# nfmoore/databricks-kubernetes-mlops-poc

Measured on AMD Instinct MI355X. Metric: requests/sec (whole node), credit-default /score, bs=1024, higher is better.
Workload: dtype fp32; 1 GPU; model=RandomForest 500xdepth16 + IForest100 + TabularDrift, global_batch=1024, request_rows=1024, with_drift=True, train_rows=20000, parallelism=dp1, device=cuda

## Files before the change

csrc/creditcore_kernels.hip:

```cpp

#include <torch/extension.h>

#include <c10/hip/HIPGuard.h>
#include <c10/hip/HIPStream.h>
#include <hip/hip_runtime.h>

#define BLOCK 256
#define N_CAT 9
#define N_NUM 14
#define MAX_DRIFT_ROWS 16384
static constexpr size_t KS_LDS_BYTES_MAX = 160 * 1024 - 1024;

#define HIP_CHECK(expr)                                              \
  do {                                                               \
    hipError_t _e = (expr);                                          \
    TORCH_CHECK(_e == hipSuccess, "HIP error: ", hipGetErrorString(_e)); \
  } while (0)


template <bool DIRECT>
__global__ __launch_bounds__(BLOCK) void forest_kernel(
    const short* __restrict__ codes,
    const float* __restrict__ nums,
    const float* __restrict__ medians,
    const int4* __restrict__ nodes,
    const int* __restrict__ tree_off,
    int n_trees,
    const int* __restrict__ feat_col,
    const int* __restrict__ feat_code,
    int n_rows,
    double* __restrict__ acc)
{
  __shared__ short s_codes[N_CAT * BLOCK];
  __shared__ float s_nums[N_NUM * BLOCK];

  const int tid = threadIdx.x;
  const int row = blockIdx.x * BLOCK + tid;
  if (row < n_rows) {
    if (!DIRECT) {
#pragma unroll
      for (int c = 0; c < N_CAT; ++c) s_codes[c * BLOCK + tid] = codes[row * N_CAT + c];
    }
#pragma unroll
    for (int c = 0; c < N_NUM; ++c) {
      const float v = nums[row * N_NUM + c];
      s_nums[c * BLOCK + tid] = isnan(v) ? medians[c] : v;
    }
  }
  if (row >= n_rows) return;

  double local = 0.0;
  for (int t = blockIdx.y; t < n_trees; t += gridDim.y) {
    const int base = tree_off[t];
    int4 nd = nodes[base];
    while (nd.x >= 0) {
      float v;
      if (DIRECT) {
        v = s_nums[nd.x * BLOCK + tid];
      } else {
        const int col = feat_col[nd.x];
        const int code = feat_code[nd.x];
        v = (code >= 0) ? ((s_codes[col * BLOCK + tid] == (short)code) ? 1.0f : 0.0f)
                        : s_nums[col * BLOCK + tid];
      }
      const float thr = __int_as_float(nd.y);
      nd = nodes[base + ((v <= thr) ? nd.z : nd.w)];
    }
    local += (double)__int_as_float(nd.y);
  }
  atomicAdd(&acc[row], local);
}

template <bool DIRECT>
__global__ __launch_bounds__(BLOCK) void forest_kernel_ilp(
    const short* __restrict__ codes,
    const float* __restrict__ nums,
    const float* __restrict__ medians,
    const int4* __restrict__ nodes,
    const int* __restrict__ tree_off,
    int n_trees,
    const int* __restrict__ feat_col,
    const int* __restrict__ feat_code,
    int n_rows,
    double* __restrict__ acc)
{
  __shared__ short s_codes[N_CAT * BLOCK];
  __shared__ float s_nums[N_NUM * BLOCK];
  const int tid = threadIdx.x;
// ... 832 lines not shown
  for (int i = threadIdx.x; i < m; i += blockDim.x) {
    float v = nums[i * n_cols + j];
    if (isnan(v)) v = medians[j];
    s_vals[i] = v;
  }
  const int64_t ref_lo = rs_off[j];
  const int n = (int)(rs_off[j + 1] - ref_lo);
  const float* __restrict__ ref = ref_sorted + ref_lo;
  __syncthreads();

  const int per = (m + gridDim.y - 1) / gridDim.y;
  const int e0 = blockIdx.y * per;
  const int e1 = min(m, e0 + per);

  double dmax = 0.0;
  for (int i = e0 + threadIdx.x; i < e1; i += blockDim.x) {
    const float x = s_vals[i];
    int lt = 0, le = 0;
    int k = 0;
    for (; k + 3 < m; k += 4) {
      const float v0 = s_vals[k], v1 = s_vals[k + 1];
      const float v2 = s_vals[k + 2], v3 = s_vals[k + 3];
      lt += (int)(v0 < x) + (int)(v1 < x) + (int)(v2 < x) + (int)(v3 < x);
      le += (int)(v0 <= x) + (int)(v1 <= x) + (int)(v2 <= x) + (int)(v3 <= x);
    }
    for (; k < m; ++k) {
      const float v = s_vals[k];
      lt += (int)(v < x);
      le += (int)(v <= x);
    }
    int l = 0, r = n;
    while (l < r) {
      const int mid = (l + r) >> 1;
      if (ref[mid] < x) l = mid + 1; else r = mid;
    }
    const int sl = l;
    r = n;
    while (l < r) {
      const int mid = (l + r) >> 1;
      if (ref[mid] <= x) l = mid + 1; else r = mid;
    }
    const int sr = l;
    const double fl = fabs((double)sl / n - (double)lt / m);
    const double fr = fabs((double)sr / n - (double)le / m);
    dmax = fmax(dmax, fmax(fl, fr));
  }

#pragma unroll
  for (int off = 32; off > 0; off >>= 1)
    dmax = fmax(dmax, __shfl_down(dmax, off, 64));
  __syncthreads();
  float* s_red = s_vals;
  const int wave = threadIdx.x >> 6;
  if ((threadIdx.x & 63) == 0) s_red[wave] = (float)dmax;
  __syncthreads();
  if (threadIdx.x == 0) {
    float d = s_red[0];
    for (int w = 1; w < (int)(blockDim.x >> 6); ++w) d = fmaxf(d, s_red[w]);
    scratch[(int64_t)j * gridDim.y + blockIdx.y] = d;
  }
}

__global__ __launch_bounds__(64) void ks_count_reduce_kernel(
    const float* __restrict__ scratch,
    int g, int n_cols,
    float* __restrict__ ks_d)
{
  const int j = blockIdx.x * 64 + threadIdx.x;
  if (j >= n_cols) return;
  float d = 0.0f;
  for (int k = 0; k < g; ++k) d = fmaxf(d, scratch[(int64_t)j * g + k]);
  ks_d[j] = d;
}

inline int ks_mb_blocks(int b) {
  int g = (b + 127) / 128;
  if (g < 1) g = 1;
  if (g > 128) g = 128;
  return g;
}
constexpr int KS_MB_MAX_G = 128;


namespace {

inline int ceil_div(int a, int b) { return (a + b - 1) / b; }

void check_inputs(const torch::Tensor& codes, const torch::Tensor& nums) {
  TORCH_CHECK(codes.is_cuda() && nums.is_cuda(), "inputs must be on GPU");
  TORCH_CHECK(codes.scalar_type() == torch::kInt16, "codes must be int16");
  TORCH_CHECK(nums.scalar_type() == torch::kFloat32, "nums must be float32");
  TORCH_CHECK(codes.is_contiguous() && nums.is_contiguous(), "inputs must be contiguous");
  TORCH_CHECK(codes.size(1) == N_CAT && nums.size(1) == N_NUM, "bad feature counts");
  TORCH_CHECK(codes.size(0) == nums.size(0), "row count mismatch");
}

}

std::vector<torch::Tensor> score_forest_pipeline(
    torch::Tensor codes, torch::Tensor nums,
    torch::Tensor cls_nodes, torch::Tensor cls_off,
    torch::Tensor feat_col, torch::Tensor feat_code,
    torch::Tensor medians, int64_t n_onehot,
    torch::Tensor if_nodes, torch::Tensor if_off,
    double if_denom, double if_offset, double if_threshold)
{
  (void)n_onehot;
  check_inputs(codes, nums);
  const int B = (int)codes.size(0);
  const int t_cls = (int)cls_off.size(0) - 1;
  const int t_if = (int)if_off.size(0) - 1;

  auto opts_f64 = torch::TensorOptions().dtype(torch::kFloat64).device(codes.device());
  auto cls_acc = torch::zeros({B}, opts_f64);
  auto if_acc = torch::zeros({B}, opts_f64);
  auto proba = torch::empty({B}, opts_f64);
  auto iscore = torch::empty({B}, opts_f64);
  auto outlier = torch::empty({B}, opts_f64);

  hipStream_t stream = c10::hip::getCurrentHIPStream();
  const int row_blocks = ceil_div(B, BLOCK);
  auto tree_chunks = [&](int t) {
    int c = ceil_div(2048, row_blocks);
    return std::max(1, std::min(c, t));
  };

  dim3 g_cls(row_blocks, tree_chunks(t_cls));
  hipLaunchKernelGGL((forest_kernel<false>), g_cls, dim3(BLOCK), 0, stream,
      codes.data_ptr<short>(), nums.data_ptr<float>(), medians.data_ptr<float>(),
      reinterpret_cast<const int4*>(cls_nodes.data_ptr<int>()),
      cls_off.data_ptr<int>(), t_cls,
      feat_col.data_ptr<int>(), feat_code.data_ptr<int>(),
      B, cls_acc.data_ptr<double>());

  dim3 g_if(row_blocks, tree_chunks(t_if));
  hipLaunchKernelGGL((forest_kernel<true>), g_if, dim3(BLOCK), 0, stream,
      codes.data_ptr<short>(), nums.data_ptr<float>(), medians.data_ptr<float>(),
      reinterpret_cast<const int4*>(if_nodes.data_ptr<int>()),
      if_off.data_ptr<int>(), t_if,
      nullptr, nullptr,
      B, if_acc.data_ptr<double>());

  hipLaunchKernelGGL(finalize_kernel, dim3(row_blocks), dim3(BLOCK), 0, stream,
      cls_acc.data_ptr<double>(), if_acc.data_ptr<double>(), B,
      0, 1.0 / (double)t_cls, 0.0, if_denom, if_offset, if_threshold,
      proba.data_ptr<double>(), iscore.data_ptr<double>(), outlier.data_ptr<double>());
  HIP_CHECK(hipGetLastError());

  return {proba, iscore, outlier};
}

torch::Tensor forest_contrib(
    torch::Tensor codes, torch::Tensor nums,
    torch::Tensor cls_nodes, torch::Tensor cls_node_value,
    torch::Tensor cls_off,
    torch::Tensor feat_col, torch::Tensor feat_code,
    torch::Tensor medians, int64_t cls_kind, int64_t block_target)
{
  check_inputs(codes, nums);
  TORCH_CHECK(block_target >= 1 && block_target <= 65535, "bad block_target");
  auto on_dev = [&](const torch::Tensor& t, torch::ScalarType st, const char* name) {
    TORCH_CHECK(t.is_cuda() && t.device() == codes.device(), name,
                " must be on the inputs' GPU");
    TORCH_CHECK(t.scalar_type() == st && t.is_contiguous(), name,
                " has the wrong dtype or is not contiguous");
  };
// ... 1201 lines not shown
#pragma unroll
  for (int off = 32; off > 0; off >>= 1)
    dmax = fmax(dmax, __shfl_down(dmax, off, 64));
  if ((threadIdx.x & 63) == 0 && dmax > 0.0)
    atomicMax(&ks_bits[j], __float_as_uint((float)dmax));
}

torch::Tensor ks_stats_sorted(
    torch::Tensor xs_sorted, torch::Tensor ref_sorted, torch::Tensor rs_off)
{
  TORCH_CHECK(xs_sorted.is_cuda() && xs_sorted.scalar_type() == torch::kFloat32
              && xs_sorted.is_contiguous());
  const int F = (int)xs_sorted.size(0);
  const int B = (int)xs_sorted.size(1);
  TORCH_CHECK((int)rs_off.size(0) == F + 1, "rs_off size mismatch");
  auto bits = torch::zeros({F},
      torch::TensorOptions().dtype(torch::kInt32).device(xs_sorted.device()));
  hipStream_t stream = c10::hip::getCurrentHIPStream();
  auto rs_off64 = rs_off.to(torch::kInt64);
  hipLaunchKernelGGL(ks_scan_kernel, dim3(F, ceil_div(B, BLOCK)), dim3(BLOCK), 0, stream,
      xs_sorted.data_ptr<float>(), F, B,
      ref_sorted.data_ptr<float>(), rs_off64.data_ptr<int64_t>(),
      reinterpret_cast<unsigned int*>(bits.data_ptr<int>()));
  HIP_CHECK(hipGetLastError());
  return bits.view(torch::kFloat32);
}

torch::Tensor ks_stats(
    torch::Tensor nums, torch::Tensor medians,
    torch::Tensor ref_sorted, torch::Tensor rs_off,
    int64_t block, int64_t ref_lds)
{
  TORCH_CHECK(nums.is_cuda() && nums.scalar_type() == torch::kFloat32 && nums.is_contiguous());
  const int B = (int)nums.size(0);
  const int F = (int)nums.size(1);
  TORCH_CHECK(B <= MAX_DRIFT_ROWS, "K-S batch too large: ", B);
  TORCH_CHECK((int)rs_off.size(0) == F + 1, "rs_off size mismatch");
  TORCH_CHECK(block == 256 || block == 512, "block must be 256 or 512");
  auto ks_d = torch::empty({F},
      torch::TensorOptions().dtype(torch::kFloat32).device(nums.device()));
  hipStream_t stream = c10::hip::getCurrentHIPStream();
  int m_pow2 = (int)block / 64;
  while (m_pow2 < B) m_pow2 <<= 1;
  size_t smem = (size_t)m_pow2 * sizeof(float);
  auto rs_off64 = rs_off.to(torch::kInt64);
  if (ref_lds) {
    int64_t maxr = 0;
    auto ro = rs_off64.cpu();
    auto* rp = ro.data_ptr<int64_t>();
    for (int j = 0; j < F; ++j) maxr = std::max<int64_t>(maxr, rp[j + 1] - rp[j]);
    smem += (size_t)maxr * sizeof(float);
    TORCH_CHECK(smem <= KS_LDS_BYTES_MAX, "ref too large for LDS");
  }
  if (block == 512)
    hipLaunchKernelGGL((ks_kernel_t<512>), dim3(F), dim3(512), smem, stream,
        nums.data_ptr<float>(), medians.data_ptr<float>(), F, B, m_pow2,
        (int)ref_lds, ref_sorted.data_ptr<float>(),
        rs_off64.data_ptr<int64_t>(), ks_d.data_ptr<float>());
  else
    hipLaunchKernelGGL((ks_kernel_t<256>), dim3(F), dim3(256), smem, stream,
        nums.data_ptr<float>(), medians.data_ptr<float>(), F, B, m_pow2,
        (int)ref_lds, ref_sorted.data_ptr<float>(),
        rs_off64.data_ptr<int64_t>(), ks_d.data_ptr<float>());
  HIP_CHECK(hipGetLastError());
  return ks_d;
}


inline bool spin_sync_enabled() {
  static const bool on = (std::getenv("CREDITCORE_BLOCK_SYNC") == nullptr);
  return on;
}

inline void sync_stream(hipStream_t s) {
  if (spin_sync_enabled()) {
    hipError_t e;
    while ((e = hipStreamQuery(s)) == hipErrorNotReady) {}
    if (e != hipSuccess) HIP_CHECK(e);
  } else {
    HIP_CHECK(hipStreamSynchronize(s));
  }
}

inline void sync_event(hipEvent_t ev) {
  static const bool spin = (std::getenv("CREDITCORE_SPIN_EVENT") != nullptr);
  if (spin) {
    hipError_t e;
    while ((e = hipEventQuery(ev)) == hipErrorNotReady) {}
    if (e != hipSuccess) HIP_CHECK(e);
  } else {
    HIP_CHECK(hipEventSynchronize(ev));
  }
}

struct ScoreSession {
  torch::Tensor cls_nodes, cls_off, feat_col, feat_code, medians;
  torch::Tensor if_nodes, if_off, ref_sorted, rs_off, cat_off;
  torch::Tensor d_codes, d_nums, acc, outs, d_drift, d_ks_scratch;
  size_t drift_bytes = 0, drift_ksd_off = 0;
  torch::Tensor pin_codes, pin_nums, pin_outs, pin_drift;
  torch::Tensor pin_hist, pin_ksd;
  double if_denom{}, if_offset{}, if_threshold{};
  int cls_kind{};
  double cls_bias{};
  int64_t total_bins{}, t_cls{}, t_if{}, capacity{};
  int device_index{};
  hipStream_t stream{};
  hipStream_t stream2{};
  hipEvent_t ev_fork{}, ev_join{};
  hipEvent_t ev_done[2]{};

  int16_t* p_codes(int s) { return pin_codes.data_ptr<int16_t>() + (size_t)s * capacity * N_CAT; }
  float* p_nums(int s) { return pin_nums.data_ptr<float>() + (size_t)s * capacity * N_NUM; }
  double* p_outs(int s) { return pin_outs.data_ptr<double>() + (size_t)s * 3 * capacity; }
  uint8_t* p_drift(int s) { return pin_drift.data_ptr<uint8_t>() + (size_t)s * drift_bytes; }
  int32_t* p_hist(int s) { return reinterpret_cast<int32_t*>(p_drift(s)); }
  float* p_ksd(int s) { return reinterpret_cast<float*>(p_drift(s) + drift_ksd_off); }
  int32_t* d_hist() { return reinterpret_cast<int32_t*>(d_drift.data_ptr<uint8_t>()); }
  float* d_ksd() { return reinterpret_cast<float*>(d_drift.data_ptr<uint8_t>() + drift_ksd_off); }

  ScoreSession(py::dict model, int64_t cap, int dev) : capacity(cap), device_index(dev) {
    c10::hip::HIPGuard guard((c10::DeviceIndex)dev);
    auto devopt = torch::TensorOptions().device(torch::kCUDA, dev);
    auto up_i32 = [&](const char* k) {
      return py::cast<torch::Tensor>(model[k]).to(devopt.dtype(torch::kInt32)).contiguous();
    };
    auto up_f32 = [&](const char* k) {
      return py::cast<torch::Tensor>(model[k]).to(devopt.dtype(torch::kFloat32)).contiguous();
    };
    cls_nodes = up_i32("cls_nodes");
    cls_off = up_i32("cls_tree_offsets");
    feat_col = up_i32("feat_col");
    feat_code = up_i32("feat_code");
    medians = up_f32("medians");
    if_nodes = up_i32("if_nodes");
    if_off = up_i32("if_tree_offsets");
    ref_sorted = up_f32("ref_sorted");
    rs_off = py::cast<torch::Tensor>(model["ref_sorted_offsets"])
                 .to(devopt.dtype(torch::kInt64)).contiguous();
    cat_off = up_i32("ref_cat_offsets");
    if (model.contains("cls_kind")) cls_kind = py::cast<int>(model["cls_kind"]);
    if (model.contains("cls_bias")) cls_bias = py::cast<double>(model["cls_bias"]);
    if_denom = py::cast<double>(model["if_denom"]);
    if_offset = py::cast<double>(model["if_offset"]);
    if_threshold = py::cast<double>(model["if_threshold"]);
    t_cls = cls_off.size(0) - 1;
    t_if = if_off.size(0) - 1;
    total_bins = py::cast<torch::Tensor>(model["ref_cat_offsets"])[-1].item<int64_t>();

    d_codes = torch::empty({capacity, N_CAT}, devopt.dtype(torch::kInt16));
    d_nums = torch::empty({capacity, N_NUM}, devopt.dtype(torch::kFloat32));
    acc = torch::zeros({2, capacity}, devopt.dtype(torch::kFloat64));
    outs = torch::empty({3, capacity}, devopt.dtype(torch::kFloat64));
    drift_ksd_off = (size_t)total_bins * sizeof(int32_t);
    drift_bytes = drift_ksd_off + (size_t)N_NUM * sizeof(float);
    d_drift = torch::empty({(int64_t)drift_bytes}, devopt.dtype(torch::kUInt8));
    d_ks_scratch = torch::empty({(int64_t)N_NUM * KS_MB_MAX_G},
                                devopt.dtype(torch::kFloat32));

    auto pinned = torch::TensorOptions().pinned_memory(true);
    pin_codes = torch::empty({2, capacity, N_CAT}, pinned.dtype(torch::kInt16));
    pin_nums = torch::empty({2, capacity, N_NUM}, pinned.dtype(torch::kFloat32));
    pin_outs = torch::empty({2, 3, capacity}, pinned.dtype(torch::kFloat64));
    pin_drift = torch::empty({2, (int64_t)drift_bytes}, pinned.dtype(torch::kUInt8));
    pin_hist = pin_drift.slice(1, 0, (int64_t)drift_ksd_off).view(torch::kInt32);
    pin_ksd = pin_drift.slice(1, (int64_t)drift_ksd_off, (int64_t)drift_bytes)
                  .view(torch::kFloat32);

    auto rs = py::cast<torch::Tensor>(model["ref_sorted_offsets"]);
    auto rs_acc = rs.accessor<int32_t, 1>();
    for (int j = 0; j + 1 < rs.size(0); ++j)
      max_ref_len = std::max(max_ref_len, (int64_t)(rs_acc[j + 1] - rs_acc[j]));

    (void)hipFuncSetAttribute(reinterpret_cast<const void*>(&ks_kernel_t<256>),
        hipFuncAttributeMaxDynamicSharedMemorySize, (int)KS_LDS_BYTES);
    (void)hipFuncSetAttribute(reinterpret_cast<const void*>(&ks_kernel_t<512>),
        hipFuncAttributeMaxDynamicSharedMemorySize, (int)KS_LDS_BYTES);
    (void)hipFuncSetAttribute(
        reinterpret_cast<const void*>(&ks_count_mb_kernel_t<512>),
        hipFuncAttributeMaxDynamicSharedMemorySize, (int)KS_LDS_BYTES);

    HIP_CHECK(hipStreamCreateWithFlags(&stream, hipStreamNonBlocking));
    HIP_CHECK(hipStreamCreateWithFlags(&stream2, hipStreamNonBlocking));
    HIP_CHECK(hipEventCreateWithFlags(&ev_fork, hipEventDisableTiming));
    HIP_CHECK(hipEventCreateWithFlags(&ev_join, hipEventDisableTiming));
    HIP_CHECK(hipEventCreateWithFlags(&ev_done[0], hipEventDisableTiming));
    HIP_CHECK(hipEventCreateWithFlags(&ev_done[1], hipEventDisableTiming));
    HIP_CHECK(hipDeviceSynchronize());
  }

  ~ScoreSession() {
    if (stream) {
      (void)hipStreamSynchronize(stream);
      for (auto& kv : graphs) (void)hipGraphExecDestroy(kv.second);
      (void)hipStreamDestroy(stream);
      (void)hipStreamDestroy(stream2);
      (void)hipEventDestroy(ev_fork);
      (void)hipEventDestroy(ev_join);
      (void)hipEventDestroy(ev_done[0]);
      (void)hipEventDestroy(ev_done[1]);
    }
  }

  void record(int b, bool with_drift, int slot) {
    HIP_CHECK(hipMemcpyAsync(d_codes.data_ptr(), p_codes(slot),
        (size_t)b * N_CAT * sizeof(short), hipMemcpyHostToDevice, stream));
    HIP_CHECK(hipMemcpyAsync(d_nums.data_ptr(), p_nums(slot),
        (size_t)b * N_NUM * sizeof(float), hipMemcpyHostToDevice, stream));
    const bool fork_drift = with_drift && b > 64;
    hipStream_t sdrift = fork_drift ? stream2 : stream;
    if (fork_drift) {
      HIP_CHECK(hipEventRecord(ev_fork, stream));
      HIP_CHECK(hipStreamWaitEvent(stream2, ev_fork, 0));
    }
    double* acc_cls = acc.data_ptr<double>();
    double* acc_if = acc_cls + b;

    const int row_blocks = ceil_div(b, BLOCK);
    auto chunks = [&](int64_t t) {
      return std::max(1, std::min(ceil_div(2048, row_blocks), (int)((t + 1) / 2)));
    };
    const int c_cls = chunks(t_cls);
    const int c_if = chunks(t_if);
    hipLaunchKernelGGL(forest_kernel_dual, dim3(row_blocks, c_cls + c_if),
        dim3(BLOCK), 0, stream,
        d_codes.data_ptr<short>(), d_nums.data_ptr<float>(), medians.data_ptr<float>(),
        reinterpret_cast<const int4*>(cls_nodes.data_ptr<int>()),
        cls_off.data_ptr<int>(), (int)t_cls,
        feat_col.data_ptr<int>(), feat_code.data_ptr<int>(),
        reinterpret_cast<const int4*>(if_nodes.data_ptr<int>()),
        if_off.data_ptr<int>(), (int)t_if, c_cls, b, acc_cls, acc_if);

    double* proba = outs.data_ptr<double>();
    hipLaunchKernelGGL(finalize_kernel, dim3(row_blocks), dim3(BLOCK), 0, stream,
        acc_cls, acc_if, b, cls_kind, 1.0 / (double)t_cls, cls_bias,
        if_denom, if_offset, if_threshold,
        proba, proba + b, proba + 2 * b);

    if (with_drift) {
      const int hist_blocks = (b <= 2048) ? 1 : std::min(row_blocks, 1024);
      if (hist_blocks > 1)
        HIP_CHECK(hipMemsetAsync(d_hist(), 0, (size_t)total_bins * sizeof(int), sdrift));
      hipLaunchKernelGGL(cat_hist_kernel, dim3(hist_blocks), dim3(BLOCK),
          (size_t)total_bins * sizeof(int), sdrift,
          d_codes.data_ptr<short>(), b, cat_off.data_ptr<int>(), (int)total_bins,
          d_hist());
      if (b <= KS_COUNT_MAX_ROWS) {
        const size_t smem = (size_t)std::max(b, 512 / 64) * sizeof(float);
        hipLaunchKernelGGL((ks_count_kernel_t<512>), dim3(N_NUM), dim3(512),
            smem, sdrift,
            d_nums.data_ptr<float>(), medians.data_ptr<float>(), N_NUM, b,
            ref_sorted.data_ptr<float>(), rs_off.data_ptr<int64_t>(), d_ksd());
      } else if (std::getenv("CREDITCORE_KS_BITONIC") != nullptr) {
        int m_pow2 = 512 / 64;
        while (m_pow2 < b) m_pow2 <<= 1;
        hipLaunchKernelGGL((ks_kernel_t<512>), dim3(N_NUM), dim3(512),
            (size_t)m_pow2 * sizeof(float), sdrift,
            d_nums.data_ptr<float>(), medians.data_ptr<float>(), N_NUM, b,
            m_pow2, 0, ref_sorted.data_ptr<float>(),
            rs_off.data_ptr<int64_t>(), d_ksd());
      } else {
        const int g = ks_mb_blocks(b);
        const size_t smem = (size_t)std::max(b, 512 / 64) * sizeof(float);
        hipLaunchKernelGGL((ks_count_mb_kernel_t<512>), dim3(N_NUM, g),
            dim3(512), smem, sdrift,
            d_nums.data_ptr<float>(), medians.data_ptr<float>(), N_NUM, b,
            ref_sorted.data_ptr<float>(), rs_off.data_ptr<int64_t>(),
            d_ks_scratch.data_ptr<float>());
        hipLaunchKernelGGL(ks_count_reduce_kernel, dim3(1), dim3(64), 0,
            sdrift, d_ks_scratch.data_ptr<float>(), g, N_NUM, d_ksd());
      }
      HIP_CHECK(hipMemcpyAsync(p_drift(slot), d_drift.data_ptr<uint8_t>(),
          drift_bytes, hipMemcpyDeviceToHost, sdrift));
      if (fork_drift) HIP_CHECK(hipEventRecord(ev_join, sdrift));
    }
    HIP_CHECK(hipMemcpyAsync(p_outs(slot), proba,
        (size_t)(3 * b) * sizeof(double), hipMemcpyDeviceToHost, stream));
    if (fork_drift) HIP_CHECK(hipStreamWaitEvent(stream, ev_join, 0));
    HIP_CHECK(hipGetLastError());
  }

  void score(int64_t b64, bool with_drift, bool sync, int64_t slot64) {
    TORCH_CHECK(b64 >= 1 && b64 <= capacity, "batch out of range: ", b64);
    TORCH_CHECK(!with_drift || b64 <= MAX_DRIFT_ROWS, "drift batch too large: ", b64);
    TORCH_CHECK(slot64 == 0 || slot64 == 1, "slot must be 0/1");
    const int b = (int)b64;
    const int slot = (int)slot64;
    py::gil_scoped_release nogil;
    c10::hip::HIPGuard guard((c10::DeviceIndex)device_index);

    const uint64_t key = ((uint64_t)b << 2) | ((with_drift ? 1u : 0u) << 1) | (uint64_t)slot;
    const bool graphable = ((b & (b - 1)) == 0) || (b % 256 == 0);
    auto it = graphs.find(key);
    if (it == graphs.end()) {
      if (!graphable || graphs.size() >= 128) {
        record(b, with_drift, slot);
        if (sync) sync_stream(stream);
        else HIP_CHECK(hipEventRecord(ev_done[slot], stream));
        return;
      }
      hipGraph_t graph;
      HIP_CHECK(hipStreamBeginCapture(stream, hipStreamCaptureModeThreadLocal));
      record(b, with_drift, slot);
      HIP_CHECK(hipStreamEndCapture(stream, &graph));
      hipGraphExec_t exec;
      HIP_CHECK(hipGraphInstantiate(&exec, graph, nullptr, nullptr, 0));
      HIP_CHECK(hipGraphDestroy(graph));
      it = graphs.emplace(key, exec).first;
    }
    HIP_CHECK(hipGraphLaunch(it->second, stream));
    if (sync) sync_stream(stream);
    else HIP_CHECK(hipEventRecord(ev_done[slot], stream));
  }

  void wait_slot(int64_t slot) {
    py::gil_scoped_release nogil;
    sync_event(ev_done[slot & 1]);
  }

  std::unordered_map<uint64_t, hipGraphExec_t> graphs;
  int64_t max_ref_len{};
  static constexpr size_t KS_LDS_BYTES = KS_LDS_BYTES_MAX;

  void synchronize() {
    py::gil_scoped_release nogil;
    HIP_CHECK(hipStreamSynchronize(stream));
  }
};


#include <pybind11/numpy.h>

#include <cmath>
#include <string>
#include <unordered_map>
#include <vector>

namespace py = pybind11;

py::tuple encode_records(py::list recs, py::list vocabs, py::list cat_names,
                         py::list num_names, py::str missing_cat) {
  const ssize_t b = py::len(recs);
  const int ncat = (int)py::len(cat_names);
  const int nnum = (int)py::len(num_names);
  py::array_t<int16_t> codes({b, (ssize_t)ncat});
  py::array_t<float> nums({b, (ssize_t)nnum});
  auto* cp = codes.mutable_data();
  auto* fp = nums.mutable_data();

  std::vector<std::unordered_map<std::string, int16_t>> maps(ncat);
  std::vector<int16_t> missing_code(ncat, -1);
  const std::string miss = py::cast<std::string>(missing_cat);
  for (int j = 0; j < ncat; ++j) {
    py::list v = vocabs[j];
    for (ssize_t k = 0; k < py::len(v); ++k)
      maps[j][py::cast<std::string>(v[k])] = (int16_t)k;
    auto it = maps[j].find(miss);
    if (it != maps[j].end()) missing_code[j] = it->second;
  }
  std::vector<PyObject*> ckeys(ncat), nkeys(nnum);
  for (int j = 0; j < ncat; ++j) ckeys[j] = PyList_GET_ITEM(cat_names.ptr(), (ssize_t)j);
  for (int j = 0; j < nnum; ++j) nkeys[j] = PyList_GET_ITEM(num_names.ptr(), (ssize_t)j);

  for (ssize_t i = 0; i < b; ++i) {
    PyObject* r = PyList_GET_ITEM(recs.ptr(), i);
    if (!PyDict_Check(r)) throw py::type_error("record must be a dict");
    for (int j = 0; j < ncat; ++j) {
      PyObject* v = PyDict_GetItem(r, ckeys[j]);
      int16_t code;
      if (v == nullptr || v == Py_None) {
        code = missing_code[j];
      } else if (PyUnicode_Check(v)) {
        Py_ssize_t len;
        const char* s = PyUnicode_AsUTF8AndSize(v, &len);
        auto it = maps[j].find(std::string(s, (size_t)len));
        code = (it == maps[j].end()) ? (int16_t)-1 : it->second;
      } else if (PyFloat_Check(v) && std::isnan(PyFloat_AS_DOUBLE(v))) {
        code = missing_code[j];
      } else {
        throw py::value_error("categorical field must be a string/None");
      }
      cp[i * ncat + j] = code;
    }
    for (int j = 0; j < nnum; ++j) {
      PyObject* v = PyDict_GetItem(r, nkeys[j]);
      float x;
// ... 693 lines not shown
  int64_t nb = (int64_t)b;
  if ((int64_t)b <= cap) {
    s.score((int64_t)b, true, true, 0);
  } else {
    s.score(cap, true, true, 0);
    s.score((int64_t)b, false, true, 0);
    nb = cap;
  }

  double pv[N_CAT + N_NUM];
  drift_pvals_raw(s.p_hist(0), s.p_ksd(0), N_NUM,
                  ref_cat_counts.data(), cat_offsets.data(),
                  (int)cat_offsets.size() - 1, n_ref, nb, pv);

  std::string out;
  {
    py::gil_scoped_release nogil;
    const double* proba = s.p_outs(0);
    const double* outlier = proba + 2 * b;
    out.reserve(b * 24 + 2048);
    out += "{\"predictions\": [";
    for (size_t i = 0; i < b; ++i) {
      if (i) out += ", ";
      append_double(out, proba[i]);
    }
    out += "], \"outliers\": [";
    for (size_t i = 0; i < b; ++i) {
      if (i) out += ", ";
      out += (outlier[i] != 0.0) ? "1.0" : "0.0";
    }
    out += "], \"feature_drift_batch\": {";
    for (int j = 0; j < nf; ++j) {
      if (j) out += ", ";
      out += '\"';
      out += names[j];
      out += "\": ";
      append_double(out, (double)(1.0f - (float)pv[j]));
    }
    out += "}}";
  }
  return py::make_tuple(py::bytes(out), (int64_t)b);
}

void submit_arrays(ScoreSession& s, py::array_t<int16_t> codes,
                   py::array_t<float> nums, int64_t slot, bool with_drift,
                   bool sync) {
  TORCH_CHECK(codes.ndim() == 2 && codes.shape(1) == N_CAT, "codes must be [B, N_CAT]");
  TORCH_CHECK(nums.ndim() == 2 && nums.shape(1) == N_NUM, "nums must be [B, N_NUM]");
  const int64_t b = codes.shape(0);
  TORCH_CHECK(nums.shape(0) == b, "codes/nums row mismatch");
  TORCH_CHECK(b >= 1 && b <= s.capacity, "batch out of range: ", b);
  auto c = codes.unchecked<2>();
  auto n = nums.unchecked<2>();
  const int sl = (int)(slot & 1);
  {
    py::gil_scoped_release nogil;
    int16_t* pc = s.p_codes(sl);
    float* pn = s.p_nums(sl);
    if (codes.strides(0) == (ssize_t)(N_CAT * sizeof(int16_t)) &&
        codes.strides(1) == (ssize_t)sizeof(int16_t)) {
      std::memcpy(pc, c.data(0, 0), (size_t)b * N_CAT * sizeof(int16_t));
    } else {
      for (int64_t i = 0; i < b; ++i)
        for (int j = 0; j < N_CAT; ++j) pc[i * N_CAT + j] = c(i, j);
    }
    if (nums.strides(0) == (ssize_t)(N_NUM * sizeof(float)) &&
        nums.strides(1) == (ssize_t)sizeof(float)) {
      std::memcpy(pn, n.data(0, 0), (size_t)b * N_NUM * sizeof(float));
    } else {
      for (int64_t i = 0; i < b; ++i)
        for (int j = 0; j < N_NUM; ++j) pn[i * N_NUM + j] = n(i, j);
    }
  }
  s.score(b, with_drift, sync, sl);
}

py::bytes response_epilogue(ScoreSession& s, int64_t slot64, int64_t b64,
                            py::array_t<int32_t> ref_cat_counts,
                            py::array_t<int32_t> cat_offsets, int64_t n_ref,
                            py::list feature_names) {
  const int slot = (int)slot64 & 1;
  const int64_t b = b64;
  TORCH_CHECK(b >= 1 && b <= s.capacity, "batch out of range: ", b);
  const int nf = (int)py::len(feature_names);
  std::vector<std::string> names(nf);
  for (int j = 0; j < nf; ++j) names[j] = py::cast<std::string>(feature_names[j]);
  const int64_t nb = std::min<int64_t>(b, MAX_DRIFT_ROWS);

  double pv[N_CAT + N_NUM];
  std::string out;
  {
    py::gil_scoped_release nogil;
    sync_event(s.ev_done[slot]);
    drift_pvals_raw(s.p_hist(slot), s.p_ksd(slot), N_NUM,
                    ref_cat_counts.data(), cat_offsets.data(),
                    (int)cat_offsets.size() - 1, n_ref, nb, pv);
    const double* proba = s.p_outs(slot);
    const double* outlier = proba + 2 * b;
    out.reserve((size_t)b * 24 + 2048);
    out += "{\"predictions\": [";
    for (int64_t i = 0; i < b; ++i) {
      if (i) out += ", ";
      append_double(out, proba[i]);
    }
    out += "], \"outliers\": [";
    for (int64_t i = 0; i < b; ++i) {
      if (i) out += ", ";
      out += (outlier[i] != 0.0) ? "1.0" : "0.0";
    }
    out += "], \"feature_drift_batch\": {";
    for (int j = 0; j < nf; ++j) {
      if (j) out += ", ";
      out += '\"';
      out += names[j];
      out += "\": ";
      append_double(out, (double)(1.0f - (float)pv[j]));
    }
    out += "}}";
  }
  return py::bytes(out);
}

PYBIND11_MODULE(TORCH_EXTENSION_NAME, m) {
  m.def("score_forest_pipeline", &score_forest_pipeline,
        "Forest classifier + isolation forest scoring (gfx950)");
  m.def("forest_contrib", &forest_contrib,
        "Per-row prediction-path feature attributions f64[B,23] (gfx950)",
        py::arg("codes"), py::arg("nums"), py::arg("cls_nodes"),
        py::arg("cls_node_value"), py::arg("cls_off"), py::arg("feat_col"),
        py::arg("feat_code"), py::arg("medians"), py::arg("cls_kind"),
        py::arg("block_target") = 512);
  m.def("forest_shap", &forest_shap,
        "Per-row exact TreeSHAP feature attributions f64[B,23] (gfx950)",
        py::arg("codes"), py::arg("nums"), py::arg("leaf_value"),
        py::arg("leaf_off"), py::arg("splits"), py::arg("medians"),
        py::arg("cls_kind"), py::arg("n_trees"),
        py::arg("block_target") = 2048);
  m.def("forest_ishap", &forest_ishap,
        "Per-row interventional Shapley values f64[B,23] against a "
        "background sample (gfx950)",
        py::arg("codes"), py::arg("nums"), py::arg("bg_codes"),
        py::arg("bg_nums"), py::arg("leaf_value"), py::arg("leaf_off"),
        py::arg("splits"), py::arg("medians"), py::arg("cls_kind"),
        py::arg("n_trees"), py::arg("block_target") = 2048);
  m.attr("ISHAP_MAX_BACKGROUND") = py::int_(ISHAP_MAX_BACKGROUND);
  m.def("hgbt_hist", &hgbt_hist,
        "HistGBT level histogram i64[n_nodes,3,total_bins] of int32 "
        "fixed-point gradients (gfx950)",
        py::arg("bins"), py::arg("bin_off"), py::arg("grp_off"),
        py::arg("node"), py::arg("gq"), py::arg("hq"), py::arg("n_nodes"),
        py::arg("total_bins"), py::arg("lds_entries"),
        py::arg("rows_per_block") = HGBT_MAX_ROWS_PER_BLOCK);
  m.def("hgbt_split", &hgbt_split,
        "HistGBT best split per open node, i64[n_nodes,9] records (gfx950)",
        py::arg("hist"), py::arg("bin_off"), py::arg("lam"), py::arg("min_leaf"));
  m.def("hgbt_split_mono", &hgbt_split_mono,
        "HistGBT best split per open node under monotone constraints: feature "
        "signs i32[F], per-node weight bounds f64[n_nodes,2] (gfx950)",
        py::arg("hist"), py::arg("bin_off"), py::arg("lam"), py::arg("min_leaf"),
        py::arg("mono"), py::arg("bounds"));
  m.def("hgbt_route", &hgbt_route,
        "HistGBT: move rows to their child node or leaf, in place (gfx950)",
        py::arg("bins"), py::arg("table"), py::arg("node"));
  m.attr("HGBT_SHIFT") = py::int_(HGBT_SHIFT);
  m.attr("HGBT_MAX_ROWS_PER_BLOCK") = py::int_(HGBT_MAX_ROWS_PER_BLOCK);
  m.attr("HGBT_LDS_BYTES_MAX") = py::int_(HGBT_LDS_BYTES_MAX);
  m.def("hrf_hist", &hrf_hist,
        "HistForest level histogram i64[n_slots,2,total_bins] of a tree batch "
        "(gfx950)",
        py::arg("bins"), py::arg("bin_off"), py::arg("grp_off"), py::arg("y"),
        py::arg("w"), py::arg("node"), py::arg("slot_off"), py::arg("n_slots"),
        py::arg("total_bins"), py::arg("lds_entries"),
        py::arg("rows_per_block") = HRF_MAX_ROWS_PER_BLOCK);
  m.def("hrf_split", &hrf_split,
        "HistForest chosen split per open slot, i64[n_slots,7] records (gfx950)",
        py::arg("hist"), py::arg("bin_off"), py::arg("slot_meta"),
        py::arg("max_features"), py::arg("min_leaf"), py::arg("seed"));
  m.def("hrf_route", &hrf_route,
        "HistForest: move the rows of every tree of the batch, in place (gfx950)",
        py::arg("bins"), py::arg("table"), py::arg("node"), py::arg("slot_off"));
  m.attr("HRF_MAX_ROWS_PER_BLOCK") = py::int_(HRF_MAX_ROWS_PER_BLOCK);
  m.attr("HRF_MAX_FEATS") = py::int_(HRF_MAX_FEATS);
  m.def("drift_stats", &drift_stats,
        "Per-feature drift statistics: categorical histograms + K-S D (gfx950)");
  m.def("encode_records", &encode_records,
        "Native request encoder: list[dict] -> (codes i16[B,9], nums f32[B,14])");
  m.def("encode_json", &encode_json,
        "Parse a /score JSON request body straight into (codes, nums)");
  py::class_<JsonEncoderState>(m, "JsonEncoder")
      .def(py::init<py::list, py::list, py::list, py::str,
                    py::array_t<int16_t>, py::array_t<float>>())
      .def("encode", [](const JsonEncoderState& st, py::bytes body) {
        return encode_json_impl(st, body);
      });
  m.def("dense_score", &dense_score,
        "Fused impute + logistic linear score + robust-z outlier (gfx950)");
  m.def("impute_transpose", &impute_transpose,
        "Fused NaN->median impute + transpose [B,F] -> [F,B] (gfx950)");
  m.def("ks_stats_sorted", &ks_stats_sorted,
        "Exact K-S D per column for pre-sorted batch columns (gfx950)");
  m.def("forest_ilp_bench", &forest_ilp_bench,
        "A/B: forest traversal, 1 vs 2 trees per thread");
  m.def("ks_stats", &ks_stats,
        "Exact two-sample K-S D per column, any column count (gfx950)",
        py::arg("nums"), py::arg("medians"), py::arg("ref_sorted"),
        py::arg("rs_off"), py::arg("block") = 256, py::arg("ref_lds") = 0);
  m.def("build_response_json", &build_response_json,
        "Serialize the /score response to JSON bytes (C, shortest doubles)");
  m.def("build_response_json_arrays", &build_response_json_arrays,
        "Serialize a /score response from plain arrays (merged-flush slices)");
  m.def("drift_pvals_host", &drift_pvals_host,
        "Drift p-values from kernel statistics (chi2 + Pelz-Good K-S), host C");
  py::class_<ScoreSession>(m, "ScoreSession")
      .def(py::init<py::dict, int64_t, int>(), py::arg("model"),
           py::arg("capacity"), py::arg("device_index"))
      .def("score", &ScoreSession::score, py::arg("b"),
           py::arg("with_drift") = true, py::arg("sync") = true,
           py::arg("slot") = 0)
      .def("wait_slot", &ScoreSession::wait_slot)
      .def("submit_arrays", &submit_arrays, py::arg("codes"), py::arg("nums"),
           py::arg("slot") = 0, py::arg("with_drift") = true,
           py::arg("sync") = false)
      .def("response_epilogue", &response_epilogue, py::arg("slot"),
           py::arg("b"), py::arg("ref_cat_counts"), py::arg("cat_offsets"),
           py::arg("n_ref"), py::arg("feature_names"))
      .def("synchronize", &ScoreSession::synchronize)
      .def("score_json_full", &score_json_full, py::arg("body"),
           py::arg("encoder"), py::arg("ref_cat_counts"),
           py::arg("cat_offsets"), py::arg("n_ref"), py::arg("feature_names"),
           py::arg("drift_cap") = -1)
      .def_readonly("capacity", &ScoreSession::capacity)
      .def_property_readonly("pin_codes", [](ScoreSession& s) { return s.pin_codes; })
      .def_property_readonly("pin_nums", [](ScoreSession& s) { return s.pin_nums; })
      .def_property_readonly("pin_outs", [](ScoreSession& s) { return s.pin_outs; })
      .def_property_readonly("pin_hist", [](ScoreSession& s) { return s.pin_hist; })
      .def_property_readonly("pin_ksd", [](ScoreSession& s) { return s.pin_ksd; });
}
```

Measured before the change: 9153 requests/s.

## Fuse forest, isolation forest, drift histogram and K-S into one kernel

Adds a single persistent-style kernel whose blocks take different roles: one block builds the categorical drift histogram, a set of blocks computes K-S statistics per numeric column slice, and the rest walk classifier and isolation-forest tree chunks. The last block per row group finalizes probabilities and outlier flags through atomic tickets. This replaces the multi-kernel, two-stream schedule with one launch per batch, cutting launch and inter-kernel dependency overhead. It also caches converted feature-name strings across response calls. The risks are load imbalance, since the K-S role does an O(m^2) in-LDS rank count, and the correctness of the atomic ticket finalization.

Result: no change. 9186 requests/s, median of 2 (+0.4%).

```diff
diff --git a/csrc/creditcore_kernels.hip b/csrc/creditcore_kernels.hip
--- a/csrc/creditcore_kernels.hip
+++ b/csrc/creditcore_kernels.hip
@@ -4,6 +4,9 @@
 #include <c10/hip/HIPGuard.h>
 #include <c10/hip/HIPStream.h>
 #include <hip/hip_runtime.h>
+
+#include <cstdlib>
+#include <cstring>
 
 #define BLOCK 256
 #define N_CAT 9
@@ -1002,6 +1005,215 @@
 constexpr int KS_MB_MAX_G = 128;
 
 
+constexpr int FUSED_MAX_ROWS = 2048;
+constexpr int FUSED_CODES_BYTES = N_CAT * BLOCK * (int)sizeof(short);
+constexpr int FUSED_LDS_BYTES = FUSED_CODES_BYTES + N_NUM * BLOCK * (int)sizeof(float);
+static_assert(FUSED_MAX_ROWS * sizeof(float) <= N_NUM * BLOCK * sizeof(float),
+              "a K-S column must fit the forest role's s_nums");
+static_assert(FUSED_CODES_BYTES % 16 == 0, "s_nums stays 16-B aligned");
+
+struct ScoreFusedArgs {
+  const short* codes;
+  const float* nums;
+  const float* medians;
+  const int4* cls_nodes;
+  const int* cls_off;
+  const int* feat_col;
+  const int* feat_code;
+  const int4* if_nodes;
+  const int* if_off;
+  int t_cls, t_if, c_cls, c_if;
+  int row_blocks, n_rows;
+  double* acc_cls;
+  double* acc_if;
+  unsigned* row_tickets;
+  int cls_kind;
+  double inv_n_trees, cls_bias, if_denom, if_offset, if_threshold;
+  double* proba;
+  double* iscore;
+  double* outlier;
+  int n_drift_blocks;
+  int ks_g;
+  const int* cat_off;
+  int total_bins;
+  int* hist;
+  const float* ref_sorted;
+  const int64_t* rs_off;
+  unsigned* ks_bits;
+  unsigned* ks_tickets;
+  float* ks_d;
+};
+
+__device__ __forceinline__ void fused_hist_role(const ScoreFusedArgs& a, int* s_hist)
+{
+  int* s_off = s_hist + a.total_bins;
+  for (int i = threadIdx.x; i < a.total_bins; i += BLOCK) s_hist[i] = 0;
+  if (threadIdx.x <= N_CAT) s_off[threadIdx.x] = a.cat_off[threadIdx.x];
+  __syncthreads();
+  for (int r = threadIdx.x; r < a.n_rows; r += BLOCK) {
+#pragma unroll
+    for (int c = 0; c < N_CAT; ++c) {
+      const int lo = s_off[c];
+      const int nbins = s_off[c + 1] - lo;
+      const int code = a.codes[r * N_CAT + c];
+      const int bin = (code < 0) ? (nbins - 1) : code;
+      atomicAdd(&s_hist[lo + bin], 1);
+    }
+  }
+  __syncthreads();
+  for (int i = threadIdx.x; i < a.total_bins; i += BLOCK) a.hist[i] = s_hist[i];
+}
+
+__device__ __forceinline__ void fused_ks_role(const ScoreFusedArgs& a, int j, int slice,
+                                              float* s_vals)
+{
+  const int m = a.n_rows;
+  for (int i = threadIdx.x; i < m; i += BLOCK) {
+    float v = a.nums[i * N_NUM + j];
+    if (isnan(v)) v = a.medians[j];
+    s_vals[i] = v;
+  }
+  const int64_t ref_lo = a.rs_off[j];
+  const int n = (int)(a.rs_off[j + 1] - ref_lo);
+  const float* __restrict__ ref = a.ref_sorted + ref_lo;
+  __syncthreads();
+
+  const int per = (m + a.ks_g - 1) / a.ks_g;
+  const int e0 = slice * per;
+  const int e1 = min(m, e0 + per);
+
+  double dmax = 0.0;
+  for (int i = e0 + threadIdx.x; i < e1; i += BLOCK) {
+    const float x = s_vals[i];
+    int lt = 0, le = 0;
+    int k = 0;
+    for (; k + 3 < m; k += 4) {
+      const float v0 = s_vals[k], v1 = s_vals[k + 1];
+      const float v2 = s_vals[k + 2], v3 = s_vals[k + 3];
+      lt += (int)(v0 < x) + (int)(v1 < x) + (int)(v2 < x) + (int)(v3 < x);
+      le += (int)(v0 <= x) + (int)(v1 <= x) + (int)(v2 <= x) + (int)(v3 <= x);
+    }
+    for (; k < m; ++k) {
+      const float v = s_vals[k];
+      lt += (int)(v < x);
+      le += (int)(v <= x);
+    }
+    int l = 0, r = n;
+    while (l < r) {
+      const int mid = (l + r) >> 1;
+      if (ref[mid] < x) l = mid + 1; else r = mid;
+    }
+    const int sl = l;
+    r = n;
+    while (l < r) {
+      const int mid = (l + r) >> 1;
+      if (ref[mid] <= x) l = mid + 1; else r = mid;
+    }
+    const int sr = l;
+    const double fl = fabs((double)sl / n - (double)lt / m);
+    const double fr = fabs((double)sr / n - (double)le / m);
+    dmax = fmax(dmax, fmax(fl, fr));
+  }
+
+#pragma unroll
+  for (int off = 32; off > 0; off >>= 1)
+    dmax = fmax(dmax, __shfl_down(dmax, off, 64));
+  __syncthreads();
+  float* s_red = s_vals;
+  if ((threadIdx.x & 63) == 0) s_red[threadIdx.x >> 6] = (float)dmax;
+  __syncthreads();
+  if (threadIdx.x == 0) {
+    float d = s_red[0];
+    for (int w = 1; w < BLOCK / 64; ++w) d = fmaxf(d, s_red[w]);
+    __hip_atomic_fetch_max(&a.ks_bits[j], __float_as_uint(d), __ATOMIC_RELAXED,
+                           __HIP_MEMORY_SCOPE_AGENT);
+    asm volatile("s_waitcnt vmcnt(0)" ::: "memory");
+    const unsigned t = __hip_atomic_fetch_add(&a.ks_tickets[j], 1u, __ATOMIC_RELAXED,
+                                              __HIP_MEMORY_SCOPE_AGENT);
+    if (t == (unsigned)a.ks_g - 1u) {
+      const unsigned bits = __hip_atomic_exchange(&a.ks_bits[j], 0u, __ATOMIC_RELAXED,
+                                                  __HIP_MEMORY_SCOPE_AGENT);
+      a.ks_d[j] = __uint_as_float(bits);
+      __hip_atomic_store(&a.ks_tickets[j], 0u, __ATOMIC_RELAXED, __HIP_MEMORY_SCOPE_AGENT);
+    }
+  }
+}
+
+__global__ __launch_bounds__(BLOCK) void score_fused_kernel(const ScoreFusedArgs a)
+{
+  __shared__ __align__(16) unsigned char s_raw[FUSED_LDS_BYTES];
+  const int tid = threadIdx.x;
+  int blk = blockIdx.x;
+  if (blk < a.n_drift_blocks) {
+    if (blk == 0) {
+      fused_hist_role(a, reinterpret_cast<int*>(s_raw));
+    } else {
+      blk -= 1;
+      fused_ks_role(a, blk % N_NUM, blk / N_NUM, reinterpret_cast<float*>(s_raw));
+    }
+    return;
+  }
+  blk -= a.n_drift_blocks;
+
+  short* s_codes = reinterpret_cast<short*>(s_raw);
+  float* s_nums = reinterpret_cast<float*>(s_raw + FUSED_CODES_BYTES);
+  const int rb = blk % a.row_blocks;
+  const int chunk = blk / a.row_blocks;
+  const int row = rb * BLOCK + tid;
+  const bool live = row < a.n_rows;
+  const bool is_cls = chunk < a.c_cls;
+  if (live) {
+    if (is_cls) {
+#pragma unroll
+      for (int c = 0; c < N_CAT; ++c) s_codes[c * BLOCK + tid] = a.codes[row * N_CAT + c];
+    }
+#pragma unroll
+    for (int c = 0; c < N_NUM; ++c) {
+      const float v = a.nums[row * N_NUM + c];
+      s_nums[c * BLOCK + tid] = isnan(v) ? a.medians[c] : v;
+    }
+    if (is_cls) {
+      const double local = forest_walk_ilp2<false>(
+          s_codes, s_nums, tid, a.cls_nodes, a.cls_off, a.t_cls, a.feat_col, a.feat_code,
+          chunk, a.c_cls);
+      atomicAdd(&a.acc_cls[row], local);
+    } else {
+      const double local = forest_walk_ilp2<true>(
+          s_codes, s_nums, tid, a.if_nodes, a.if_off, a.t_if, nullptr, nullptr,
+          chunk - a.c_cls, a.c_if);
+      atomicAdd(&a.acc_if[row], local);
+    }
+  }
+  asm volatile("s_waitcnt vmcnt(0)" ::: "memory");
+  __syncthreads();
+  int* s_last = reinterpret_cast<int*>(s_raw);
+  if (tid == 0) {
+    const unsigned t = __hip_atomic_fetch_add(&a.row_tickets[rb], 1u, __ATOMIC_RELAXED,
+                                              __HIP_MEMORY_SCOPE_AGENT);
+    *s_last = (t == (unsigned)(a.c_cls + a.c_if) - 1u) ? 1 : 0;
+  }
+  __syncthreads();
+  if (*s_last == 0) return;
+
+  if (live) {
+    const double cls_sum = __longlong_as_double((long long)__hip_atomic_exchange(
+        reinterpret_cast<unsigned long long*>(&a.acc_cls[row]), 0ull, __ATOMIC_RELAXED,
+        __HIP_MEMORY_SCOPE_AGENT));
+    const double if_sum = __longlong_as_double((long long)__hip_atomic_exchange(
+        reinterpret_cast<unsigned long long*>(&a.acc_if[row]), 0ull, __ATOMIC_RELAXED,
+        __HIP_MEMORY_SCOPE_AGENT));
+    a.proba[row] = a.cls_kind ? 1.0 / (1.0 + exp(-(cls_sum + a.cls_bias)))
+                              : cls_sum * a.inv_n_trees;
+    const double anomaly = exp2(-if_sum / a.if_denom);
+    const double s = anomaly + a.if_offset;
+    a.iscore[row] = s;
+    a.outlier[row] = (s > a.if_threshold) ? 1.0 : 0.0;
+  }
+  if (tid == 0)
+    __hip_atomic_store(&a.row_tickets[rb], 0u, __ATOMIC_RELAXED, __HIP_MEMORY_SCOPE_AGENT);
+}
+
+
 namespace {
 
 inline int ceil_div(int a, int b) { return (a + b - 1) / b; }
@@ -2369,6 +2581,14 @@
   }
 }
 
+inline bool score_fused_default() {
+  static const bool on = [] {
+    const char* v = std::getenv("CREDITCORE_SCORE_FUSED");
+    return v == nullptr || std::strcmp(v, "0") != 0;
+  }();
+  return on;
+}
+
 inline void sync_event(hipEvent_t ev) {
   static const bool spin = (std::getenv("CREDITCORE_SPIN_EVENT") != nullptr);
   if (spin) {
@@ -2384,6 +2604,10 @@
   torch::Tensor cls_nodes, cls_off, feat_col, feat_code, medians;
   torch::Tensor if_nodes, if_off, ref_sorted, rs_off, cat_off;
   torch::Tensor d_codes, d_nums, acc, outs, d_drift, d_ks_scratch;
+  torch::Tensor d_fused_sync;
+  bool fused{};
+  py::object names_src;
+  std::vector<std::string> names_cache;
   size_t drift_bytes = 0, drift_ksd_off = 0;
   torch::Tensor pin_codes, pin_nums, pin_outs, pin_drift;
   torch::Tensor pin_hist, pin_ksd;
@@ -2406,7 +2630,11 @@
   int32_t* d_hist() { return reinterpret_cast<int32_t*>(d_drift.data_ptr<uint8_t>()); }
   float* d_ksd() { return reinterpret_cast<float*>(d_drift.data_ptr<uint8_t>() + drift_ksd_off); }
 
-  ScoreSession(py::dict model, int64_t cap, int dev) : capacity(cap), device_index(dev) {
+  ScoreSession(py::dict model, int64_t cap, int dev)
+      : ScoreSession(model, cap, dev, score_fused_default()) {}
+
+  ScoreSession(py::dict model, int64_t cap, int dev, bool fused_path)
+      : fused(fused_path), capacity(cap), device_index(dev) {
     c10::hip::HIPGuard guard((c10::DeviceIndex)dev);
     auto devopt = torch::TensorOptions().device(torch::kCUDA, dev);
     auto up_i32 = [&](const char* k) {
@@ -2444,6 +2672,10 @@
     d_drift = torch::empty({(int64_t)drift_bytes}, devopt.dtype(torch::kUInt8));
     d_ks_scratch = torch::empty({(int64_t)N_NUM * KS_MB_MAX_G},
                                 devopt.dtype(torch::kFloat32));
+    d_fused_sync = torch::zeros({(int64_t)ceil_div((int)capacity, BLOCK) + 2 * N_NUM},
+                                devopt.dtype(torch::kInt32));
+    if ((size_t)(total_bins + N_CAT + 1) * sizeof(int) > (size_t)FUSED_LDS_BYTES)
+      fused = false;
 
     auto pinned = torch::TensorOptions().pinned_memory(true);
     pin_codes = torch::empty({2, capacity, N_CAT}, pinned.dtype(torch::kInt16));
@@ -2567,6 +2799,68 @@
     HIP_CHECK(hipGetLastError());
   }
 
+  bool use_fused(int b) const { return fused && b <= FUSED_MAX_ROWS; }
+
+  void record_fused(int b, bool with_drift, int slot) {
+    HIP_CHECK(hipMemcpyAsync(d_codes.data_ptr(), p_codes(slot),
+        (size_t)b * N_CAT * sizeof(short), hipMemcpyHostToDevice, stream));
+    HIP_CHECK(hipMemcpyAsync(d_nums.data_ptr(), p_nums(slot),
+        (size_t)b * N_NUM * sizeof(float), hipMemcpyHostToDevice, stream));
+    const int row_blocks = ceil_div(b, BLOCK);
+    auto chunks = [&](int64_t t) {
+      return std::max(1, std::min(ceil_div(2048, row_blocks), (int)((t + 1) / 2)));
+    };
+    unsigned* sync_words = reinterpret_cast<unsigned*>(d_fused_sync.data_ptr<int>());
+    const int n_tickets = ceil_div((int)capacity, BLOCK);
+    double* proba = outs.data_ptr<double>();
+    ScoreFusedArgs a{};
+    a.codes = d_codes.data_ptr<short>();
+    a.nums = d_nums.data_ptr<float>();
+    a.medians = medians.data_ptr<float>();
+    a.cls_nodes = reinterpret_cast<const int4*>(cls_nodes.data_ptr<int>());
+    a.cls_off = cls_off.data_ptr<int>();
+    a.feat_col = feat_col.data_ptr<int>();
+    a.feat_code = feat_code.data_ptr<int>();
+    a.if_nodes = reinterpret_cast<const int4*>(if_nodes.data_ptr<int>());
+    a.if_off = if_off.data_ptr<int>();
+    a.t_cls = (int)t_cls;
+    a.t_if = (int)t_if;
+    a.c_cls = chunks(t_cls);
+    a.c_if = chunks(t_if);
+    a.row_blocks = row_blocks;
+    a.n_rows = b;
+    a.acc_cls = acc.data_ptr<double>();
+    a.acc_if = a.acc_cls + b;
+    a.row_tickets = sync_words;
+    a.cls_kind = cls_kind;
+    a.inv_n_trees = 1.0 / (double)t_cls;
+    a.cls_bias = cls_bias;
+    a.if_denom = if_denom;
+    a.if_offset = if_offset;
+    a.if_threshold = if_threshold;
+    a.proba = proba;
+    a.iscore = proba + b;
+    a.outlier = proba + 2 * b;
+    a.ks_g = ks_mb_blocks(b);
+    a.n_drift_blocks = with_drift ? 1 + N_NUM * a.ks_g : 0;
+    a.cat_off = cat_off.data_ptr<int>();
+    a.total_bins = (int)total_bins;
+    a.hist = d_hist();
+    a.ref_sorted = ref_sorted.data_ptr<float>();
+    a.rs_off = rs_off.data_ptr<int64_t>();
+    a.ks_bits = sync_words + n_tickets;
+    a.ks_tickets = sync_words + n_tickets + N_NUM;
+    a.ks_d = d_ksd();
+    const int grid = a.n_drift_blocks + row_blocks * (a.c_cls + a.c_if);
+    hipLaunchKernelGGL(score_fused_kernel, dim3(grid), dim3(BLOCK), 0, stream, a);
+    if (with_drift)
+      HIP_CHECK(hipMemcpyAsync(p_drift(slot), d_drift.data_ptr<uint8_t>(),
+          drift_bytes, hipMemcpyDeviceToHost, stream));
+    HIP_CHECK(hipMemcpyAsync(p_outs(slot), proba,
+        (size_t)(3 * b) * sizeof(double), hipMemcpyDeviceToHost, stream));
+    HIP_CHECK(hipGetLastError());
+  }
+
   void score(int64_t b64, bool with_drift, bool sync, int64_t slot64) {
     TORCH_CHECK(b64 >= 1 && b64 <= capacity, "batch out of range: ", b64);
     TORCH_CHECK(!with_drift || b64 <= MAX_DRIFT_ROWS, "drift batch too large: ", b64);
@@ -2576,19 +2870,23 @@
     py::gil_scoped_release nogil;
     c10::hip::HIPGuard guard((c10::DeviceIndex)device_index);
 
-    const uint64_t key = ((uint64_t)b << 2) | ((with_drift ? 1u : 0u) << 1) | (uint64_t)slot;
+    const bool fused_now = use_fused(b);
+    const uint64_t key = ((uint64_t)b << 3) | ((fused_now ? 1u : 0u) << 2) |
+                         ((with_drift ? 1u : 0u) << 1) | (uint64_t)slot;
     const bool graphable = ((b & (b - 1)) == 0) || (b % 256 == 0);
     auto it = graphs.find(key);
     if (it == graphs.end()) {
       if (!graphable || graphs.size() >= 128) {
-        record(b, with_drift, slot);
+        if (fused_now) record_fused(b, with_drift, slot);
+        else record(b, with_drift, slot);
         if (sync) sync_stream(stream);
         else HIP_CHECK(hipEventRecord(ev_done[slot], stream));
         return;
       }
       hipGraph_t graph;
       HIP_CHECK(hipStreamBeginCapture(stream, hipStreamCaptureModeThreadLocal));
-      record(b, with_drift, slot);
+      if (fused_now) record_fused(b, with_drift, slot);
+      else record(b, with_drift, slot);
       HIP_CHECK(hipStreamEndCapture(stream, &graph));
       hipGraphExec_t exec;
       HIP_CHECK(hipGraphInstantiate(&exec, graph, nullptr, nullptr, 0));
@@ -3448,9 +3746,15 @@
   const int slot = (int)slot64 & 1;
   const int64_t b = b64;
   TORCH_CHECK(b >= 1 && b <= s.capacity, "batch out of range: ", b);
-  const int nf = (int)py::len(feature_names);
-  std::vector<std::string> names(nf);
-  for (int j = 0; j < nf; ++j) names[j] = py::cast<std::string>(feature_names[j]);
+  if (!s.names_src.is(feature_names)) {
+    std::vector<std::string> fresh(py::len(feature_names));
+    for (size_t j = 0; j < fresh.size(); ++j)
+      fresh[j] = py::cast<std::string>(feature_names[j]);
+    s.names_cache = std::move(fresh);
+    s.names_src = feature_names;
+  }
+  const std::vector<std::string>& names = s.names_cache;
+  const int nf = (int)names.size();
   const int64_t nb = std::min<int64_t>(b, MAX_DRIFT_ROWS);
 
   double pv[N_CAT + N_NUM];
@@ -3580,6 +3884,11 @@
   py::class_<ScoreSession>(m, "ScoreSession")
       .def(py::init<py::dict, int64_t, int>(), py::arg("model"),
            py::arg("capacity"), py::arg("device_index"))
+      .def(py::init<py::dict, int64_t, int, bool>(), py::arg("model"),
+           py::arg("capacity"), py::arg("device_index"), py::arg("fused"))
+      .def_readonly("fused", &ScoreSession::fused)
+      .def("uses_fused", &ScoreSession::use_fused, py::arg("b"),
+           "True when a b-row batch scores through score_fused_kernel")
       .def("score", &ScoreSession::score, py::arg("b"),
            py::arg("with_drift") = true, py::arg("sync") = true,
            py::arg("slot") = 0)
```
